# Berghojo/bmhrl

Measured on AMD Instinct MI355X. Metric: caption-train steps/sec, higher is better.
Workload: dtype bf16; 1 GPU; BMHRL warmstart step (BASELINE configs[1]): B=16/GPU Tv=256 Ta=800 L=30 V=10172 N=2 d_model=1024 H=4 dropout=0.1; global_batch=16, parallelism=dp1, launch=hip-graph

## Files before the change

### bmhrl_amd/_lib.py

```python
from __future__ import annotations

import ctypes as C
import os

_HERE = os.path.dirname(os.path.abspath(__file__))
LIB_PATH = os.environ.get("BMHRL_HIP_LIB") or os.path.join(_HERE, "csrc", "libbmhrl_hip.so")

i32, i64, u64, f32, f64 = C.c_int32, C.c_int64, C.c_uint64, C.c_float, C.c_double
ptr = C.c_void_p


class RnnLayer(C.Structure):
    _fields_ = [("w_ih", C.c_void_p), ("w_hh", C.c_void_p), ("b_ih", C.c_void_p), ("b_hh", C.c_void_p),
                ("in_seq", C.c_void_p), ("in_ld", C.c_int64), ("in_dim", C.c_int32), ("gates", C.c_int32),
                ("seq_out", C.c_void_p), ("h", C.c_void_p * 2), ("c", C.c_void_p * 2),
                ("arelu_alpha", C.c_void_p), ("arelu_beta", C.c_void_p), ("xproj", C.c_void_p)]


class FusionTailParams(C.Structure):
    _fields_ = [(n, C.c_void_p) for n in ("gamma_ca", "beta_ca", "gamma_cv", "beta_cv", "a_v",
                                          "dgamma_ca", "dbeta_ca", "dgamma_cv", "dbeta_cv", "da_v")]


class GemmDesc(C.Structure):
# ... 6 lines not shown
        ("epilogue", i32), ("alpha", f32), ("relu", i32), ("accumulate", i32), ("allow_split_k", i32),
        ("bias", ptr),
        ("residual", ptr), ("ldr", i64), ("r_sb1", i64), ("r_sb2", i64),
        ("mask", ptr), ("mask_sb1", i64), ("mask_sm", i64),
        ("rowvec", ptr), ("rowvec2", ptr), ("rv_sb1", i64), ("rv_sb2", i64),
        ("aux", ptr), ("ldaux", i64), ("aux_sb1", i64), ("aux_sb2", i64),
        ("dropout_p", f32), ("seed", u64), ("drop_sb1", i64), ("drop_sb2", i64), ("drop_sm", i64), ("seed_dev", ptr),
        ("colsum", ptr), ("colsum_sb2", i64), ("bias_sb2", i64), ("colsum_sb1", i64), ("bias_sb1", i64),
        ("split_ws", ptr), ("split_ws_elems", i64),
    ]


PROTOTYPES = {
    "bmhrl_gemm": [C.POINTER(GemmDesc), ptr],
    "bmhrl_gemm_group": [C.POINTER(GemmDesc), i32, ptr],
    "bmhrl_attention_fwd": [ptr, i64, ptr, i64, ptr, i64, ptr, i64, ptr, ptr, ptr, i64, i64, i32, i32, i32, i32, i32, f32,
                            f32, u64, ptr, ptr],
    "bmhrl_attention_shared128_fwd": [ptr, i64, ptr, i64, ptr, i64, ptr, ptr, ptr, i64, i32, i32, i32, i32, f32, ptr],
    "bmhrl_attention_fwd_f16": [ptr, i64, ptr, i64, ptr, i64, ptr, i64, ptr, ptr, ptr, i64, i64, i32, i32, i32, i32, i32, f32,
                                f32, u64, ptr, ptr],
    "bmhrl_attention_shared128_fwd_f16": [ptr, i64, ptr, i64, ptr, i64, ptr, ptr, ptr, i64, i32, i32, i32, i32, f32, ptr],
    "bmhrl_attention_shared128_bwd": [ptr, i64, ptr, i64, ptr, i64, ptr, ptr, ptr, ptr, i64, ptr, i64, ptr, i64, i32, ptr, i32, i32,
                                      i32, i32, f32, ptr],
    "bmhrl_small_attention_fwd": [ptr, i64, ptr, i64, ptr, i64, ptr, i64, ptr, i32, ptr, i64, i64, i32, i32, i32, i32, i32, f32, f32,
                                  u64, ptr, ptr],
    "bmhrl_small_attention_bwd": [ptr, i64, ptr, i32, ptr, i64, ptr, i64, ptr, i64, ptr, i64, ptr, i64, ptr, i64, ptr, ptr, ptr,
                                  ptr, i64, i64, i32, i32, i32, i32, i32, f32, ptr],
    "bmhrl_cast_memory": [ptr, ptr, ptr, i32, i32, i32, i32, ptr],
    "bmhrl_memory_attention": [i32, ptr, i64, ptr, i64, ptr, i64, i32, ptr, i64, i64, ptr, i64, ptr, i64, i32, i32, i32, i32, i32,
                               i32, f32, ptr],
    "bmhrl_softmax_rows": [ptr, i64, ptr, i64, i64, i32, i32, i64, ptr],
    "bmhrl_softmax_bwd_rows": [ptr, i64, ptr, i64, ptr, i64, i64, i32, f32, ptr, i64, i64, i32, i32, i32, i64, ptr],
    "bmhrl_attn_delta": [ptr, i64, ptr, i64, ptr, f32, i32, i32, i32, i32, ptr],
    "bmhrl_attention_bwd_scores256": [ptr, i64, ptr, i64, ptr, i64, ptr, i64, ptr, ptr, ptr, i64, ptr, ptr, i64, i32, i32, i32, i32,
                                      f32, ptr],
    "bmhrl_layernorm_fwd": [ptr, ptr, ptr, ptr, i64, ptr, ptr, ptr, i64, i32, ptr],
    "bmhrl_layernorm_bwd": [ptr, ptr, ptr, ptr, ptr, ptr, ptr, ptr, ptr, i64, i32, ptr],
    "bmhrl_layernorm_bwd_ws": [ptr, ptr, ptr, ptr, ptr, ptr, ptr, ptr, ptr, i64, i32, ptr, i64, ptr],
    "bmhrl_layernorm_fwd_groups": [ptr, ptr, ptr, ptr, i64, ptr, ptr, ptr, i64, i32, i32, ptr],
    "bmhrl_layernorm_bwd_groups": [ptr, ptr, ptr, ptr, ptr, ptr, ptr, ptr, ptr, i64, i32, i32, ptr],
    "bmhrl_add_posenc": [ptr, ptr, ptr, ptr, ptr, i64, i32, i32, i32, f32, u64, ptr, ptr],
    "bmhrl_embed_posenc": [ptr, ptr, f32, ptr, ptr, ptr, ptr, i32, i32, i32, f32, f32, u64, ptr, ptr],
    "bmhrl_embed_bwd": [ptr, ptr, f32, ptr, ptr, i32, i32, i32, f32, ptr],
    "bmhrl_cast_bf16": [ptr, i64, ptr, i64, i64, i32, f32, f32, u64, ptr, ptr],
    "bmhrl_cast_split3_bf16": [ptr, i64, ptr, i64, i64, i32, i64, i32, ptr, i64, i32, ptr],
    "bmhrl_cast_colsum_bf16": [ptr, i64, ptr, i64, i64, i32, f32, f32, u64, ptr, ptr, ptr],
# ... 149 lines not shown
```

### bmhrl_amd/csrc/attention128.hip

```cpp
#include "attention_bwd.h"

bool bmhrl_attn128_pair_ok(int B, int H, int Sq, int Sk);
int bmhrl_attn128_pair_fwd(const void* Qp, int64_t ldq, const void* X, int64_t ldx, void* ctx, int64_t ldo, float* row_max,
                           float* row_sum, const uint8_t* mask, int64_t mask_sb, int32_t B, int32_t H, int32_t Sq, int32_t Sk,
                           float scale, hipStream_t stream);

namespace {
int g_cfg128 = 0;
}

void bmhrl_attn128_set_cfg(int code) { g_cfg128 = code; }

int bmhrl_attn128_plan_fwd(int B, int H, int Sq, int Sk) {
  if (B <= 0 || H <= 0 || Sq <= 0 || Sk <= 0) return -22;
  const bool pair_served = bmhrl_attn128_pair_ok(B, H, Sq, Sk);
  const int code = g_cfg128 != 0 ? g_cfg128 : attn128_auto_code(B, H, Sq, Sk, pair_served);
  if (code == 14) return pair_served ? 14 : -22;
  if (code != 41 && code != 22 && code != 24) return -22;
  if (Sk > AttnCfg<128, 4, 1, 4, true>::MAX_SK || !attn_grid_ok(B, H, Sq, code / 10)) return -22;
  return code;
}
int bmhrl_attn128_plan_bwd(int B, int H, int Sq, int Sk) {
  if (B <= 0 || H <= 0 || Sq <= 0 || Sk <= 0 || Sk > AttnCfg<128, 4, 1, 4, true>::MAX_SK) return -22;
  const bool wide = attn128_bwd_wide(B, H, Sq);
  if (!attn_grid_ok(B, H, Sq, wide ? 4 : 2)) return -22;
  return wide ? 41 : 22;
}

extern "C" int bmhrl_attention_shared128_fwd(const void* Qp, int64_t ldq, const void* X, int64_t ldx, void* ctx, int64_t ldo,
                                             float* row_max, float* row_sum, const uint8_t* mask, int64_t mask_sb,
                                             int32_t B, int32_t H, int32_t Sq, int32_t Sk, float scale,
                                             bmhrl_stream_t stream) {
  return attention128_entry(Qp, ldq, X, ldx, ctx, ldo, row_max, row_sum, mask, mask_sb, B, H, Sq, Sk, scale, g_cfg128,
                            (hipStream_t)stream, bmhrl_attn128_pair_fwd, bmhrl_attn128_pair_ok);
}

extern "C" int64_t bmhrl_attention_shared128_bwd_workspace(int32_t B, int32_t H, int32_t Sk) {
  return (int64_t)B * H * Sk * 128;
}

extern "C" int bmhrl_attention_shared128_bwd(const void* Qp, int64_t ldq, const void* X, int64_t ldx, const void* dCx, int64_t lddo,
                                             const float* row_max, const float* row_sum, const float* delta,
                                             const uint8_t* mask, int64_t mask_sb, void* dQp, int64_t lddq, float* dX,
                                             int64_t lddx, int32_t accumulate_dx, float* workspace, int32_t B, int32_t H,
                                             int32_t Sq, int32_t Sk, float scale, bmhrl_stream_t stream) {
  constexpr int DK = 128;
  BMHRL_CHECK_ARG(Qp && X && dCx && row_max && row_sum && delta && dQp);
  BMHRL_CHECK_ARG(B > 0 && H > 0 && Sq > 0 && Sk > 0);
  BMHRL_CHECK_ARG(ldq % 8 == 0 && ldx % 8 == 0 && lddo % 8 == 0 && lddq % 8 == 0);
  BMHRL_CHECK_ARG(ldq >= (int64_t)H * DK && ldx >= DK && lddo >= (int64_t)H * DK && lddq >= (int64_t)H * DK);
  BMHRL_CHECK_ARG((((uintptr_t)Qp | (uintptr_t)X | (uintptr_t)dCx | (uintptr_t)dQp) & 15) == 0);
  BMHRL_CHECK_ARG((int64_t)Sk * ldx * 2 < (1ll << 31));
  BMHRL_CHECK_ARG(dX == nullptr || (workspace != nullptr && lddx >= DK && lddx % 4 == 0 && ((uintptr_t)dX & 15) == 0));
  AttnBwdArgs a;
  a.Q = (const bf16_t*)Qp; a.ldq = ldq; a.X = (const bf16_t*)X; a.ldx = ldx; a.dO = (const bf16_t*)dCx; a.lddo = lddo;
  a.dQ = (bf16_t*)dQp; a.lddq = lddq; a.dXp = workspace;
  a.row_max = row_max; a.row_sum = row_sum; a.delta = delta; a.mask = mask; a.mask_sb = mask_sb;
  a.B = B; a.H = H; a.Sq = Sq; a.Sk = Sk; a.scale = scale;
  hipStream_t s = (hipStream_t)stream;
  const bool wide = attn128_bwd_wide(B, H, Sq);
  const int qw = wide ? 4 : 2;
  if (Sk > AttnCfg<DK, 4, 1, 4, true>::MAX_SK) return -22;
  a.q_tiles = (Sq + 32 * qw - 1) / (32 * qw);
  BMHRL_CHECK_ARG((int64_t)B * H * a.q_tiles * H * a.q_tiles < (1ll << 32));
  a.per_b = H * a.q_tiles;
  a.map_mode = (B % 8 == 0) ? 0 : 2;
  a.magic_perb = div_magic((unsigned)a.per_b);
  a.magic_qt = div_magic((unsigned)a.q_tiles);
  a.magic_h = div_magic((unsigned)H);
  dim3 grid((unsigned)(B * H * a.q_tiles));
  if (wide) hipLaunchKernelGGL((attn_bwd_dq128_kernel<4, 1, 4>), grid, dim3(256), 0, s, a);
  else hipLaunchKernelGGL((attn_bwd_dq128_kernel<2, 2, 4>), grid, dim3(256), 0, s, a);
  if (dX != nullptr) {
    const int kblocks = (Sk + 32 * DX_WAVES - 1) / (32 * DX_WAVES);
    hipLaunchKernelGGL((attn_bwd_dx128_kernel<4>), dim3((unsigned)(B * H * kblocks)), dim3(64 * DX_WAVES), 0, s, a);
    const long total = (long)B * Sk * 32;
    hipLaunchKernelGGL(attn_bwd_dx_reduce_kernel, dim3((unsigned)((total + 255) / 256)), dim3(256), 0, s, (const float*)workspace, dX,
                       (long)lddx, B, H, Sk, accumulate_dx);
  }
  return hip_status(hipGetLastError());
}
```

### bmhrl_amd/csrc/attention_bwd.h

```cpp
#pragma once
#include "attention_fwd.h"

namespace {

template <int OFF>
__device__ __forceinline__ f32x4 asm_ldsf4(unsigned addr) {
  f32x4 r;
  asm volatile("ds_read_b128 %0, %1 offset:%2" : "=v"(r) : "v"(addr), "n"(OFF));
  return r;
}

struct AttnBwdArgs {
  const bf16_t* Q; long ldq;
  const bf16_t* X; long ldx;
  const bf16_t* dO; long lddo;
  bf16_t* dQ; long lddq;
  float* dXp;
  const float* row_max; const float* row_sum; const float* delta;
  const uint8_t* mask; long mask_sb;
  int B, H, Sq, Sk;
  float scale;
  int q_tiles, map_mode, per_b;
  unsigned magic_perb, magic_qt, magic_h;
};

template <int QW, int KW, int NS>
__global__ __launch_bounds__(64 * QW * KW, 2) void attn_bwd_dq128_kernel(const AttnBwdArgs p) {
  constexpr int DK = 128;
  using C = AttnCfg<DK, QW, KW, NS, true>;
  constexpr int NW = C::NW, NT = C::NT, BN = C::BN, VST = C::VST, ND = C::ND, NH = C::NH;
  static_assert(NS >= 3, "tile t+1 has landed at the end of iteration t while tile t+NS-1 is in flight");
  __shared__ __attribute__((aligned(16))) char smem_raw[C::LDS_BYTES];
  uint64_t* s_slow = reinterpret_cast<uint64_t*>(smem_raw + C::MAIN_BYTES);
  uint64_t* s_valid = s_slow + C::WORDS;
  bf16_t* smem = reinterpret_cast<bf16_t*>(smem_raw);
  const unsigned lds0 = (unsigned)(uintptr_t)(__attribute__((address_space(3))) char*)smem_raw;
  constexpr float LOG2E = 1.4426950408889634f;

  const int tid = threadIdx.x, lane = tid & 63;
  const int wave_s = __builtin_amdgcn_readfirstlane(tid >> 6);
  const int qi = wave_s / KW, ki = wave_s % KW;
  const int r32 = lane & 31, h = lane >> 5;
  const int g1 = (lane >> 4) & 1, q4 = (lane & 15) >> 2, p4 = lane & 3;
  int bh, qt;
  if (p.map_mode == 0) {
    const int xcd = blockIdx.x & 7, idx = blockIdx.x >> 3;
    const int q1 = fast_div(idx, p.per_b, p.magic_perb), rem = idx - q1 * p.per_b;
    const int hq = fast_div(rem, p.q_tiles, p.magic_qt);
    bh = (xcd + 8 * q1) * p.H + hq;
// ... 25 lines not shown
      static_for<0, GL>([&](auto i) {
        constexpr int I = decltype(i)::value;
        const int r = RPI * I + hi_;
        unsigned o = (unsigned)(r * (int)p.ldx * 2 + ((pch_ ^ swz(wrow + r)) << 4) - 1024 * (I & 3));
        asm volatile("" : "+v"(o));
        glds16<1024 * (I & 3)>(base + o, sdst + (I / 4) * 4 * RPI * DK);
      });
    } else {
      int hi_ = hi, pch_ = pch;
      asm volatile("" : "+v"(hi_), "+v"(pch_));
      static_for<0, GL>([&](auto i) {
        constexpr int I = decltype(i)::value;
        const int r = RPI * I + hi_;
        const int gr = min(k0 + wrow + r, p.Sk - 1);
        glds16<0>(Xgb + (unsigned)(gr * (int)p.ldx * 2 + ((pch_ ^ swz(wrow + r)) << 4)), sdst + RPI * I * DK);
      });
    }
  };
#pragma unroll
  for (int s = 0; s < NS - 1; ++s)
    if (s < nt_all) issue_x(s);

  bf16x8 qf[8], dof[8];
  {
    const long ro = ((long)b * p.Sq + (q_ok ? q_row : 0));
    const bf16_t* qp = p.Q + ro * p.ldq + hd * DK + 8 * h;
    const bf16_t* dp = p.dO + ro * p.lddo + hd * DK + 8 * h;
#pragma unroll
    for (int s = 0; s < 8; ++s) {
      qf[s] = q_ok ? *reinterpret_cast<const bf16x8*>(qp + 16 * s) : zero_bf16x8();
      dof[s] = q_ok ? *reinterpret_cast<const bf16x8*>(dp + 16 * s) : zero_bf16x8();
    }
  }
  float m2 = 0.f, invl_s = 0.f, dl_s = 0.f;
  if (q_ok) {
    const long si = ((long)b * p.H + hd) * p.Sq + q_row;
    m2 = p.row_max[si] * LOG2E;
    invl_s = p.scale / p.row_sum[si];
    dl_s = p.delta[si] * invl_s;
  }
  const int n_words = (nt_all * BN + 255) >> 8;
  for (int j = 0; j * NW < n_words; ++j) {
    const int i0 = 4 * (tid + NT * j);
    uint32_t v = 0x01010101u;
    if (mrow_b != nullptr && i0 < p.Sk) {
      if (mask_al4 && i0 + 4 <= p.Sk) {
        v = *reinterpret_cast<const uint32_t*>(mrow_b + i0);
      } else {
        v = 0;
#pragma unroll
        for (int e = 0; e < 4; ++e)
          if (i0 + e < p.Sk) v |= (uint32_t)mrow_b[i0 + e] << (8 * e);
      }
    }
    bool any_slow = false, any_valid = false;
#pragma unroll
    for (int e = 0; e < 4; ++e) {
      const bool keep = i0 + e < p.Sk && ((v >> (8 * e)) & 0xffu) != 0;
      any_slow |= !keep;
      any_valid |= keep;
    }
    const uint64_t bs = __ballot(any_slow), bv = __ballot(any_valid);
// ... 179 lines not shown
      const int srow = lane / CPRO, sch = lane % CPRO;
      const int q0 = qt * (32 * QW) + qi * 32;
      bf16x8 wout[NST];
#pragma unroll
      for (int i = 0; i < NST; ++i) wout[i] = *reinterpret_cast<const bf16x8*>(img + (RPS * i + srow) * ROWB + sch * 16);
      bf16_t* op = p.dQ + ((long)b * p.Sq + q0 + srow) * p.lddq + hd * DK + MY * 32 + sch * 8;
      const long ostep = (long)RPS * p.lddq;
#pragma unroll
      for (int i = 0; i < NST; ++i) {
        if (q0 + RPS * i + srow < p.Sq) *reinterpret_cast<bf16x8*>(op) = wout[i];
        op += ostep;
      }
    }
  });
}

constexpr int DX_WAVES = 4;
template <int NS>
struct DxCfg {
  static constexpr int TILE = 32 * 128 * 2;
  static constexpr int STAT = 3 * 64 * 4;
  static constexpr int STAGE = 2 * TILE + STAT;
  static constexpr int OUT = DX_WAVES * 32 * (512 + 16);
  static constexpr int LDS = cmax(NS * STAGE, OUT);
};

template <int NS>
__global__ __launch_bounds__(64 * DX_WAVES, 2) void attn_bwd_dx128_kernel(const AttnBwdArgs p) {
  constexpr int DK = 128;
  using C = DxCfg<NS>;
  __shared__ __attribute__((aligned(16))) char smem_raw[C::LDS];
  const unsigned lds0 = (unsigned)(uintptr_t)(__attribute__((address_space(3))) char*)smem_raw;
  constexpr float LOG2E = 1.4426950408889634f;
  const int tid = threadIdx.x, lane = tid & 63;
  const int wave_s = __builtin_amdgcn_readfirstlane(tid >> 6);
  const int r32 = lane & 31, h = lane >> 5;
  const int g1 = (lane >> 4) & 1, q4 = (lane & 15) >> 2, p4 = lane & 3;
  const int kblocks = (p.Sk + 32 * DX_WAVES - 1) / (32 * DX_WAVES);
  const int bh = blockIdx.x / kblocks, kb = blockIdx.x - bh * kblocks;
  const int b = bh / p.H, hd = bh - b * p.H;
  const int key = kb * (32 * DX_WAVES) + wave_s * 32 + r32;
  const bool key_in = key < p.Sk;
  const bool keep = key_in && (p.mask == nullptr || p.mask[(long)b * p.mask_sb + key] != 0);
  const int nqt = (p.Sq + 31) / 32;
  auto swz = [](int row) { return ((row & 3) << 2) | ((row >> 2) & 3); };

  const int hi = lane >> 4, pch = lane & 15;
// ... 9 lines not shown
      const int gr = min(q0 + r, p.Sq - 1);
      const int sc = (pch ^ swz(r)) << 4;
      __builtin_amdgcn_global_load_lds((const __attribute__((address_space(1))) void*)(Qgb + (long)gr * p.ldq * 2 + sc),
                                       (__attribute__((address_space(3))) void*)(st + (2 * wave_s + i) * 1024), 16, 0, 0);
      __builtin_amdgcn_global_load_lds((const __attribute__((address_space(1))) void*)(Dgb + (long)gr * p.lddo * 2 + sc),
                                       (__attribute__((address_space(3))) void*)(st + C::TILE + (2 * wave_s + i) * 1024), 16, 0, 0);
    }
    if (wave_s < 3) {
      const float* src = wave_s == 0 ? p.row_max : (wave_s == 1 ? p.row_sum : p.delta);
      const int gq = min(q0 + lane, p.Sq - 1);
      __builtin_amdgcn_global_load_lds((const __attribute__((address_space(1))) void*)(src + sbase + gq),
                                       (__attribute__((address_space(3))) void*)(st + 2 * C::TILE + wave_s * 256), 4, 0, 0);
    }
  };
  constexpr int PT = 5;
#pragma unroll
  for (int s = 0; s < NS - 1; ++s)
    if (s < nqt) issue(s);

  bf16x8 xf[8];
  {
    const bf16_t* xp = p.X + ((long)b * p.Sk + min(key, p.Sk - 1)) * p.ldx + 8 * h;
#pragma unroll
    for (int s = 0; s < 8; ++s) xf[s] = *reinterpret_cast<const bf16x8*>(xp + 16 * s);
  }
  f32x16 o[4];
#pragma unroll
  for (int d = 0; d < 4; ++d)
#pragma unroll
    for (int r = 0; r < 16; ++r) o[d][r] = 0.f;

  unsigned r_addr[8], t_addr[4][2];
#pragma unroll
  for (int st = 0; st < 8; ++st) r_addr[st] = lds0 + r32 * 256 + (((2 * st + h) ^ swz(r32)) << 4);
#pragma unroll
  for (int dd = 0; dd < 4; ++dd)
#pragma unroll
    for (int sec = 0; sec < 2; ++sec) {
      const int lc = 4 * dd + 2 * g1 + (p4 >> 1);
      const int pc = lc ^ ((q4 << 2) | ((h + 2 * sec) & 3));
      t_addr[dd][sec] = lds0 + (4 * h + q4) * 256 + (pc << 4) + ((p4 & 1) << 3);
    }
  const unsigned s_addr = lds0 + 2 * C::TILE + (4 * h) * 4;

  const float c_log2 = p.scale * LOG2E;
  const bool wave3 = wave_s == 3;
  asm volatile("s_waitcnt vmcnt(0)" ::: "memory");
  __builtin_amdgcn_s_barrier();
  asm volatile("" ::: "memory");
  for (int t = 0; t < nqt; ++t) {
    const bool more = t + NS - 1 < nqt;
    if (more) issue(t + NS - 1);
    const unsigned soff = (unsigned)(t % NS) * C::STAGE;
    bf16x8 af[8];
    f32x16 s_acc, dp_acc;
#pragma unroll
    for (int r = 0; r < 16; ++r) { s_acc[r] = 0.f; dp_acc[r] = 0.f; }
#pragma unroll
    for (int st = 0; st < 8; ++st) asm volatile("ds_read_b128 %0, %1 offset:0" : "=v"(af[st]) : "v"(r_addr[st] + soff));
    asm volatile("s_waitcnt lgkmcnt(0)" : "+v"(af[0]), "+v"(af[1]), "+v"(af[2]), "+v"(af[3]), "+v"(af[4]), "+v"(af[5]), "+v"(af[6]), "+v"(af[7]));
    BMHRL_SB();
    static_for<0, 8>([&](auto st_) { s_acc = __builtin_amdgcn_mfma_f32_32x32x16_bf16(af[decltype(st_)::value], xf[decltype(st_)::value], s_acc, 0, 0, 0); });
    BMHRL_SB();
#pragma unroll
    for (int st = 0; st < 8; ++st) asm volatile("ds_read_b128 %0, %1 offset:%2" : "=v"(af[st]) : "v"(r_addr[st] + soff), "n"(C::TILE));
    f32x4 smax[4], ssum[4], sdel[4];
    smax[0] = asm_ldsf4<0>(s_addr + soff);   smax[1] = asm_ldsf4<32>(s_addr + soff);
    smax[2] = asm_ldsf4<64>(s_addr + soff);  smax[3] = asm_ldsf4<96>(s_addr + soff);
    ssum[0] = asm_ldsf4<256>(s_addr + soff); ssum[1] = asm_ldsf4<288>(s_addr + soff);
    ssum[2] = asm_ldsf4<320>(s_addr + soff); ssum[3] = asm_ldsf4<352>(s_addr + soff);
    sdel[0] = asm_ldsf4<512>(s_addr + soff); sdel[1] = asm_ldsf4<544>(s_addr + soff);
    sdel[2] = asm_ldsf4<576>(s_addr + soff); sdel[3] = asm_ldsf4<608>(s_addr + soff);
    asm volatile("s_waitcnt lgkmcnt(12)" : "+v"(af[0]), "+v"(af[1]), "+v"(af[2]), "+v"(af[3]), "+v"(af[4]), "+v"(af[5]), "+v"(af[6]), "+v"(af[7]));
    BMHRL_SB();
    static_for<0, 8>([&](auto st_) { dp_acc = __builtin_amdgcn_mfma_f32_32x32x16_bf16(af[decltype(st_)::value], xf[decltype(st_)::value], dp_acc, 0, 0, 0); });
    asm volatile("s_waitcnt lgkmcnt(0)"
                 : "+v"(smax[0]), "+v"(smax[1]), "+v"(smax[2]), "+v"(smax[3]), "+v"(ssum[0]), "+v"(ssum[1]), "+v"(ssum[2]), "+v"(ssum[3]),
                   "+v"(sdel[0]), "+v"(sdel[1]), "+v"(sdel[2]), "+v"(sdel[3]));
    BMHRL_SB();
    bf16x8 tf[4][2];
    auto read_t = [&](const unsigned base) {
#pragma unroll
      for (int dd = 0; dd < 4; ++dd) {
        const unsigned a0 = t_addr[dd][0] + base, a1 = t_addr[dd][1] + base;
        tf[dd][0] = join8(asm_tr4<0>(a0), asm_tr4<8 * 256>(a1));
        tf[dd][1] = join8(asm_tr4<16 * 256>(a0), asm_tr4<24 * 256>(a1));
      }
    };
    read_t(soff + C::TILE);
    bf16x8 pb[2], dsb[2];
    const int q0 = t * 32 + 4 * h;
    const bool ragged = t * 32 + 32 > p.Sq;
#pragma unroll
    for (int g = 0; g < 4; ++g)
#pragma unroll
      for (int j = 0; j < 4; ++j) {
        const int r = 4 * g + j;
        const float rmax = smax[g][j];
        const float m2 = rmax * LOG2E;
        float invl = __builtin_amdgcn_rcpf(ssum[g][j]);
        if (ragged && q0 + 8 * g + j >= p.Sq) invl = 0.f;
        const float e = __builtin_amdgcn_exp2f(fmaf(s_acc[r], c_log2, -m2));
        const float pr = keep ? e * invl : (rmax == NEG_MASK ? invl : 0.f);
        const float dsv = keep ? pr * (dp_acc[r] - sdel[g][j]) * p.scale : 0.f;
        pb[r >> 3][r & 7] = (bf16_t)pr;
        dsb[r >> 3][r & 7] = (bf16_t)dsv;
      }
    asm volatile("s_waitcnt lgkmcnt(0)"
                 : "+v"(tf[0][0]), "+v"(tf[0][1]), "+v"(tf[1][0]), "+v"(tf[1][1]), "+v"(tf[2][0]), "+v"(tf[2][1]), "+v"(tf[3][0]), "+v"(tf[3][1]));
    BMHRL_SB();
    static_for<0, 8>([&](auto i_) {
      constexpr int I = decltype(i_)::value;
      o[I / 2] = __builtin_amdgcn_mfma_f32_32x32x16_bf16(tf[I / 2][I % 2], pb[I % 2], o[I / 2], 0, 0, 0);
    });
    BMHRL_SB();
    read_t(soff);
    asm volatile("s_waitcnt lgkmcnt(0)"
                 : "+v"(tf[0][0]), "+v"(tf[0][1]), "+v"(tf[1][0]), "+v"(tf[1][1]), "+v"(tf[2][0]), "+v"(tf[2][1]), "+v"(tf[3][0]), "+v"(tf[3][1]));
    BMHRL_SB();
    static_for<0, 8>([&](auto i_) {
      constexpr int I = decltype(i_)::value;
      o[I / 2] = __builtin_amdgcn_mfma_f32_32x32x16_bf16(tf[I / 2][I % 2], dsb[I % 2], o[I / 2], 0, 0, 0);
    });
    if (more && NS > 2) {
      if (wave3) asm volatile("s_waitcnt vmcnt(%0)" ::"n"((NS - 2) * (PT - 1)) : "memory");
      else asm volatile("s_waitcnt vmcnt(%0)" ::"n"((NS - 2) * PT) : "memory");
    } else {
      asm volatile("s_waitcnt vmcnt(0)" ::: "memory");
    }
    __builtin_amdgcn_s_barrier();
    asm volatile("" ::: "memory");
  }
  asm volatile("s_waitcnt vmcnt(0) lgkmcnt(0)" ::: "memory");
  __builtin_amdgcn_s_barrier();
  asm volatile("" ::: "memory");

  constexpr int ROWB = 512 + 16;
  char* img = smem_raw + wave_s * 32 * ROWB;
#pragma unroll
  for (int dd = 0; dd < 4; ++dd)
#pragma unroll
    for (int g = 0; g < 4; ++g) {
      f32x4 v;
#pragma unroll
      for (int j = 0; j < 4; ++j) v[j] = o[dd][4 * g + j];
      *reinterpret_cast<f32x4*>(img + r32 * ROWB + (dd * 32 + 8 * g + 4 * h) * 4) = v;
    }
  const int srow = lane >> 5, sch = lane & 31;
  const int k0 = kb * (32 * DX_WAVES) + wave_s * 32;
  float* outp = p.dXp + (((long)b * p.H + hd) * p.Sk + k0 + srow) * DK + sch * 4;
#pragma unroll
  for (int i = 0; i < 16; ++i) {
    const f32x4 v = *reinterpret_cast<const f32x4*>(img + (2 * i + srow) * ROWB + sch * 16);
    if (k0 + 2 * i + srow < p.Sk) *reinterpret_cast<f32x4*>(outp) = v;
// ... 21 lines not shown
```

### bmhrl_amd/functional.py

```python
from __future__ import annotations

import math
import itertools
import os
import weakref
from typing import Optional

import torch

from . import ops
from .ops import pad8

_BF16 = torch.bfloat16


class ShadowCache:

    def __init__(self):
        self.w = {}
        self.b = {}
        self.split = {}
        self.epoch = 0

    def invalidate(self):
# ... 744 lines not shown
        rows = B * L
        ldx, dmp, Skp = pad8(dq), pad8(dm), pad8(Sk)
        scale = 1.0 / math.sqrt(dk)
        need = ctx.needs_input_grad
        dy = dy.contiguous()
        w_q, w_k, w_v, w_o = SHADOWS.weight(wq), SHADOWS.weight(wk), SHADOWS.weight(wv), SHADOWS.weight(wo)
        zeros = torch.zeros if dmp != dm else torch.empty
        dyb, dbo = _cast_dy(dy, rows, dq, p_drop, s_res, need[11])
        dOb = torch.empty(rows, D, dtype=_BF16, device=dev)
        dbv = SCRATCH.f32(D, device=dev) if need[9] else None
        dwo, _ = _linear_bwd(dyb, ldx, rows, dq, Ob, D, D, w_o, need_dw=need[10], need_db=False, need_dx=True,
                             dx_bf16=dOb, lddxb=D, dx_drop=p_drop, dx_seed=s_attn, dx_colsum=dbv)
        dwv = None
        if need[8]:
            dwv = SCRATCH.f32(D, dm, device=dev, zero=not ops.gemm_overwrites(dk, dm, rows, H))
            ops.gemm(dOb, Cx, dk, dm, rows, lda=D, ldb=H * dmp, a_trans=True, b_trans=True, batch=(1, H), a_strides=(0, dk),
                     b_strides=(0, dmp), C_f32=dwv, ldc=dm, c_strides=(0, dk * dm), allow_split_k=True)
        dCx = zeros(rows, H * dmp, dtype=_BF16, device=dev)
        ops.gemm(dOb, w_v, rows, dm, dk, lda=D, ldb=w_v.shape[1], b_trans=True, batch=(1, H), a_strides=(0, dk),
                 b_strides=(0, dk * w_v.shape[1]), C_bf16=dCx, ldcb=H * dmp, cb_strides=(0, dmp))
        delta = None
        if flash:
            delta = torch.empty(B, H, L, device=dev)
            ops.attn_delta(dCx, H * dmp, Cx, H * dmp, delta, B, H, L, dmp)
        dQp = zeros(rows, H * dmp, dtype=_BF16, device=dev)
        dmem = None
        dxn = None
        if flash and FUSED_ATTN_BWD:
            if self_att:
                dxn = torch.empty(rows, dq, device=dev)
                target = dxn
            elif need[1]:
                dmem = torch.empty(B, Sk, dm, device=dev)
                target = dmem
            else:
                target = None
            ops.attention_shared128_bwd(Qp, memb, dCx, stats[0], stats[1], delta, m8, msb, dQp, target, False, B, H, L, Sk,
                                        scale, H * dmp, dmp, H * dmp, H * dmp, lddx=dm)
        else:
            dS = _padded_bf16(B * L * H, Sk, dev).view(B, L, H, Skp)
            pstr = (L * H * Skp, Skp)
            if flash:
                P = _padded_bf16(B * L * H, Sk, dev).view(B, L, H, Skp)
                ops.gemm(Qp, memb, L, Sk, dm, lda=H * dmp, ldb=dmp, batch=(B, H), a_strides=(L * H * dmp, dmp),
                         b_strides=(Sk * dmp, 0), C_bf16=P, ldcb=H * Skp, cb_strides=pstr, epilogue=ops.EPI_PROB, alpha=scale,
                         mask=m8, mask_sb1=msb, mask_sm=0, rowvec=stats[0], rowvec2=stats[1], rv_strides=(H * L, L))
                ops.gemm(dCx, memb, L, Sk, dm, lda=H * dmp, ldb=dmp, batch=(B, H), a_strides=(L * H * dmp, dmp),
                         b_strides=(Sk * dmp, 0), C_bf16=dS, ldcb=H * Skp, cb_strides=pstr, epilogue=ops.EPI_DSCORE, alpha=scale,
                         rowvec=delta, rv_strides=(H * L, L), aux=P, ldaux=H * Skp, aux_strides=pstr, mask=m8, mask_sb1=msb)
            else:
                P = stats[0]
                dP = torch.empty(B, L, H, Skp, device=dev)
                ops.gemm(dCx, memb, L, Sk, dm, lda=H * dmp, ldb=dmp, batch=(B, H), a_strides=(L * H * dmp, dmp),
                         b_strides=(Sk * dmp, 0), C_f32=dP, ldc=H * Skp, c_strides=pstr)
                ops.softmax_bwd_rows(P, Skp, dP, Skp, dS, Skp, B * L * H, Sk, scale, m8, msb, msq, H, L)
            def grad_mem(target, first_accumulates):
                ops.gemm(P, dCx, Sk, dm, L * H, lda=Skp, ldb=dmp, a_trans=True, b_trans=True, batch=(B, 1),
                         a_strides=(L * H * Skp, 0), b_strides=(L * H * dmp, 0), C_f32=target, ldc=dm, c_strides=(Sk * dm, 0),
                         accumulate=first_accumulates)
                ops.gemm(dS, Qp, Sk, dm, L * H, lda=Skp, ldb=dmp, a_trans=True, b_trans=True, batch=(B, 1),
                         a_strides=(L * H * Skp, 0), b_strides=(L * H * dmp, 0), C_f32=target, ldc=dm, c_strides=(Sk * dm, 0),
# ... 1246 lines not shown
```

### bmhrl_amd/ops.py

```python
from __future__ import annotations

import ctypes as C
import math
import os
from typing import Optional, Tuple

import numpy as np
import torch

from . import _lib

EPI_LINEAR, EPI_PROB, EPI_DSCORE, EPI_RELU_BWD = 0, 1, 2, 3


def pad8(n: int) -> int:
    return (n + 7) & ~7


def stream() -> int:
    return torch._C._cuda_getCurrentRawStream(torch.cuda.current_device())


_Tensor, _Parameter = torch.Tensor, torch.nn.Parameter
_TENSORS = frozenset((_Tensor, _Parameter))
# ... 187 lines not shown
def memory_attention(backward, X, x_off, ldx, mem, mem_t, ldt, PD, pd_row, pd_slot, Y, ldy, mask, mask_sb, n_mem, B2, H, L, Sk, dm,
                     scale):
    _launch("bmhrl_memory_attention", int(backward), _at(X, x_off), ldx, mem, Sk * dm, mem_t, dm * ldt, ldt, PD, pd_row, pd_slot,
            Y, ldy, mask, mask_sb, n_mem, B2, H, L, Sk, dm, scale)


def attention_shared128_fwd(Qp, X, ctx, row_max, row_sum, mask, mask_sb, B, H, Sq, Sk, scale, ldq, ldx, ldo):
    f16 = Qp.dtype == torch.float16
    if any((t.dtype == torch.float16) != f16 for t in (X, ctx)):
        raise RuntimeError("attention_shared128_fwd: Qp, X and ctx must share one 16-bit type")
    _launch("bmhrl_attention_shared128_fwd_f16" if f16 else "bmhrl_attention_shared128_fwd", Qp, ldq, X, ldx, ctx, ldo, row_max,
            row_sum, mask, mask_sb, B, H, Sq, Sk, scale)


def attention_shared128_bwd(Qp, X, dCx, row_max, row_sum, delta, mask, mask_sb, dQp, dX, accumulate_dx, B, H, Sq, Sk, scale,
                            ldq, ldx, lddo, lddq, lddx=128):
    ws = None
    if dX is not None:
        ws = torch.empty(int(_query("bmhrl_attention_shared128_bwd_workspace", B, H, Sk)), device=Qp.device)
    _launch("bmhrl_attention_shared128_bwd", Qp, ldq, X, ldx, dCx, lddo, row_max, row_sum, delta, mask, mask_sb, dQp, lddq, dX,
            lddx, int(bool(accumulate_dx)), ws, B, H, Sq, Sk, scale)


def softmax_bwd_rows(P, ldp, dP, lddp, dS, ldds, rows, cols, scale, mask=None, mask_sb=0, mask_sq=0, rows_per_query=1, queries=1,
                     rows_per_group=0, group_stride=0, p_off=0, ds_off=0):
    _launch("bmhrl_softmax_bwd_rows", _at(P, p_off), ldp, dP, lddp, _at(dS, ds_off), ldds, rows, cols, scale, mask, mask_sb,
            mask_sq, rows_per_query, queries, rows_per_group, group_stride)


def softmax_rows(S, lds, P, ldp, rows, cols, rows_per_group=0, group_stride=0, p_off=0):
    _launch("bmhrl_softmax_rows", S, lds, _at(P, p_off), ldp, rows, cols, rows_per_group, group_stride)


def attn_delta(dO, lddo, O, ldo, delta, B, H, Sq, dk, scale=1.0):
    _launch("bmhrl_attn_delta", dO, lddo, O, ldo, delta, scale, B, H, Sq, dk)


def attention_bwd_scores256_ok(Sq, Sk, dk, msq):
    return bool(_query("bmhrl_attention_bwd_scores256_ok", Sq, Sk, dk, msq))


def attention_bwd_scores256(Q, ldq, K, ldk, V, ldv, dO, lddo, row_max, row_sum, mask, msb, P, dS, ldp, B, H, Sq, Sk, scale,
                            q_off=0, k_off=0, v_off=0):
    _launch("bmhrl_attention_bwd_scores256", _at(Q, q_off), ldq, _at(K, k_off), ldk, _at(V, v_off), ldv, dO, lddo, row_max,
            row_sum, mask, msb, P, dS, ldp, B, H, Sq, Sk, scale)

# ... 964 lines not shown
```

### include/bmhrl_hip.h

```cpp
#ifndef BMHRL_HIP_H
#define BMHRL_HIP_H

#include <stdint.h>

#ifdef __cplusplus
extern "C" {
#endif

typedef void* bmhrl_stream_t;

enum {
  BMHRL_EPI_LINEAR = 0,
  BMHRL_EPI_PROB = 1,
  BMHRL_EPI_DSCORE = 2,
  BMHRL_EPI_RELU_BWD = 3
};

typedef struct bmhrl_gemm_desc {
  int32_t M, N, K;
  int32_t batch1, batch2;
  const void* A; int64_t lda, a_sb1, a_sb2; int32_t a_trans;
  const void* B; int64_t ldb, b_sb1, b_sb2; int32_t b_trans;
  float* C;  int64_t ldc, c_sb1, c_sb2;
  void* Cb;  int64_t ldcb, cb_sb1, cb_sb2;
// ... 27 lines not shown
                        void* O, int64_t ldo, float* row_max, float* row_sum, const uint8_t* mask, int64_t mask_sb,
                        int64_t mask_sq,
                        int32_t B, int32_t H, int32_t Sq, int32_t Sk, int32_t DK, float scale,
                        float dropout_p, uint64_t seed, const uint64_t* seed_dev, bmhrl_stream_t stream);

int bmhrl_attention_shared128_fwd(const void* Qp, int64_t ldq, const void* X, int64_t ldx, void* ctx, int64_t ldo,
                                  float* row_max, float* row_sum, const uint8_t* mask, int64_t mask_sb,
                                  int32_t B, int32_t H, int32_t Sq, int32_t Sk, float scale, bmhrl_stream_t stream);

int bmhrl_attention_fwd_f16(const void* Q, int64_t ldq, const void* K, int64_t ldk, const void* V, int64_t ldv,
                            void* O, int64_t ldo, float* row_max, float* row_sum, const uint8_t* mask, int64_t mask_sb,
                            int64_t mask_sq, int32_t B, int32_t H, int32_t Sq, int32_t Sk, int32_t DK, float scale,
                            float dropout_p, uint64_t seed, const uint64_t* seed_dev, bmhrl_stream_t stream);
int bmhrl_attention_shared128_fwd_f16(const void* Qp, int64_t ldq, const void* X, int64_t ldx, void* ctx, int64_t ldo,
                                      float* row_max, float* row_sum, const uint8_t* mask, int64_t mask_sb,
                                      int32_t B, int32_t H, int32_t Sq, int32_t Sk, float scale, bmhrl_stream_t stream);

int64_t bmhrl_attention_shared128_bwd_workspace(int32_t B, int32_t H, int32_t Sk);
int bmhrl_attention_shared128_bwd(const void* Qp, int64_t ldq, const void* X, int64_t ldx, const void* dCx, int64_t lddo,
                                  const float* row_max, const float* row_sum, const float* delta, const uint8_t* mask,
                                  int64_t mask_sb, void* dQp, int64_t lddq, float* dX, int64_t lddx, int32_t accumulate_dx,
                                  float* workspace, int32_t B, int32_t H, int32_t Sq, int32_t Sk, float scale,
                                  bmhrl_stream_t stream);

int bmhrl_attention_max_keys(void);

int bmhrl_attention_config(int32_t head_dim, int32_t code);

int bmhrl_attention_plan(int32_t kind, int32_t B, int32_t H, int32_t Sq, int32_t Sk, int64_t mask_sq);

int bmhrl_small_attention_ok(int32_t Sq, int32_t Sk, int32_t dk);
int bmhrl_small_attention_fwd(const void* Q, int64_t ldq, const void* K, int64_t ldk, const void* V, int64_t ldv, void* O,
                              int64_t ldo, void* P, int32_t ldp, const uint8_t* mask, int64_t mask_sb, int64_t mask_sq,
                              int32_t B, int32_t H, int32_t Sq, int32_t Sk, int32_t dk, float scale, float dropout_p,
                              uint64_t seed, const uint64_t* seed_dev, bmhrl_stream_t stream);
int bmhrl_small_attention_bwd(const void* dO, int64_t lddo, const void* P, int32_t ldp, const void* Q, int64_t ldq,
                              const void* K, int64_t ldk, const void* V, int64_t ldv, void* dQ, int64_t lddq, void* dK,
                              int64_t lddk, void* dV, int64_t lddv, float* dbq, float* dbk, float* dbv, const uint8_t* mask,
                              int64_t mask_sb, int64_t mask_sq, int32_t B, int32_t H, int32_t Sq, int32_t Sk, int32_t dk,
                              float scale, bmhrl_stream_t stream);

int bmhrl_memory_attention_ok(int32_t L, int32_t Sk, int32_t dm);
int bmhrl_cast_memory(const float* x, void* y, void* y_t, int32_t B, int32_t Sk, int32_t dm, int32_t ldt, bmhrl_stream_t stream);
int bmhrl_memory_attention(int32_t backward, const void* X, int64_t ldx, const void* mem, int64_t mem_sb, const void* mem_t,
                           int64_t mem_t_sb, int32_t ldt, void* PD, int64_t pd_row, int64_t pd_slot, void* Y, int64_t ldy,
                           const uint8_t* mask, int64_t mask_sb, int32_t n_mem, int32_t B2, int32_t H, int32_t L, int32_t Sk,
// ... 345 lines not shown
```

Before: 210.3 steps/s (one step = one B=16 batch on one GPU; whole-job aggregate over all GPUs).

## Fuse attention delta into the dQ backward kernel and simplify the dX softmax math

The shared-128 attention backward gains a context-aware variant. The dQ kernel computes the per-row delta (dO·O) itself and writes it out, so the separate attn_delta launch is skipped when FUSED_ATTN_BWD is set. The dX kernel now folds the per-row max, sum, mask and delta into combined constants staged in LDS, which removes per-element reciprocal and branch work. It also lets waves with no live keys only take part in the pipeline barriers. In exchange there are extra LDS space and writes per tile, and the new path depends on FUSED_ATTN_BWD being defined elsewhere.

```diff
diff --git a/bmhrl_amd/_lib.py b/bmhrl_amd/_lib.py
--- a/bmhrl_amd/_lib.py
+++ b/bmhrl_amd/_lib.py
@@ -52,6 +52,8 @@
     "bmhrl_attention_shared128_fwd_f16": [ptr, i64, ptr, i64, ptr, i64, ptr, ptr, ptr, i64, i32, i32, i32, i32, f32, ptr],
     "bmhrl_attention_shared128_bwd": [ptr, i64, ptr, i64, ptr, i64, ptr, ptr, ptr, ptr, i64, ptr, i64, ptr, i64, i32, ptr, i32, i32,
                                       i32, i32, f32, ptr],
+    "bmhrl_attention_shared128_bwd_ctx": [ptr, i64, ptr, i64, ptr, i64, ptr, i64, ptr, ptr, ptr, ptr, i64, ptr, i64, ptr, i64, i32,
+                                          ptr, i32, i32, i32, i32, f32, ptr],
     "bmhrl_small_attention_fwd": [ptr, i64, ptr, i64, ptr, i64, ptr, i64, ptr, i32, ptr, i64, i64, i32, i32, i32, i32, i32, f32, f32,
                                   u64, ptr, ptr],
     "bmhrl_small_attention_bwd": [ptr, i64, ptr, i32, ptr, i64, ptr, i64, ptr, i64, ptr, i64, ptr, i64, ptr, i64, ptr, ptr, ptr,
diff --git a/bmhrl_amd/csrc/attention128.hip b/bmhrl_amd/csrc/attention128.hip
--- a/bmhrl_amd/csrc/attention128.hip
+++ b/bmhrl_amd/csrc/attention128.hip
@@ -39,23 +39,26 @@
   return (int64_t)B * H * Sk * 128;
 }
 
-extern "C" int bmhrl_attention_shared128_bwd(const void* Qp, int64_t ldq, const void* X, int64_t ldx, const void* dCx, int64_t lddo,
-                                             const float* row_max, const float* row_sum, const float* delta,
-                                             const uint8_t* mask, int64_t mask_sb, void* dQp, int64_t lddq, float* dX,
-                                             int64_t lddx, int32_t accumulate_dx, float* workspace, int32_t B, int32_t H,
-                                             int32_t Sq, int32_t Sk, float scale, bmhrl_stream_t stream) {
+namespace {
+int attention128_bwd(const void* Qp, int64_t ldq, const void* X, int64_t ldx, const void* dCx, int64_t lddo, const void* Cx,
+                     int64_t ldcx, const float* row_max, const float* row_sum, float* delta, const uint8_t* mask,
+                     int64_t mask_sb, void* dQp, int64_t lddq, float* dX, int64_t lddx, int32_t accumulate_dx, float* workspace,
+                     int32_t B, int32_t H, int32_t Sq, int32_t Sk, float scale, bmhrl_stream_t stream) {
   constexpr int DK = 128;
+  const bool ctx = Cx != nullptr;
   BMHRL_CHECK_ARG(Qp && X && dCx && row_max && row_sum && delta && dQp);
   BMHRL_CHECK_ARG(B > 0 && H > 0 && Sq > 0 && Sk > 0);
   BMHRL_CHECK_ARG(ldq % 8 == 0 && ldx % 8 == 0 && lddo % 8 == 0 && lddq % 8 == 0);
   BMHRL_CHECK_ARG(ldq >= (int64_t)H * DK && ldx >= DK && lddo >= (int64_t)H * DK && lddq >= (int64_t)H * DK);
   BMHRL_CHECK_ARG((((uintptr_t)Qp | (uintptr_t)X | (uintptr_t)dCx | (uintptr_t)dQp) & 15) == 0);
+  BMHRL_CHECK_ARG(!ctx || (ldcx % 8 == 0 && ldcx >= (int64_t)H * DK && ((uintptr_t)Cx & 15) == 0));
   BMHRL_CHECK_ARG((int64_t)Sk * ldx * 2 < (1ll << 31));
   BMHRL_CHECK_ARG(dX == nullptr || (workspace != nullptr && lddx >= DK && lddx % 4 == 0 && ((uintptr_t)dX & 15) == 0));
   AttnBwdArgs a;
   a.Q = (const bf16_t*)Qp; a.ldq = ldq; a.X = (const bf16_t*)X; a.ldx = ldx; a.dO = (const bf16_t*)dCx; a.lddo = lddo;
   a.dQ = (bf16_t*)dQp; a.lddq = lddq; a.dXp = workspace;
   a.row_max = row_max; a.row_sum = row_sum; a.delta = delta; a.mask = mask; a.mask_sb = mask_sb;
+  a.Cx = (const bf16_t*)Cx; a.ldcx = ldcx; a.delta_out = delta;
   a.B = B; a.H = H; a.Sq = Sq; a.Sk = Sk; a.scale = scale;
   hipStream_t s = (hipStream_t)stream;
   const bool wide = attn128_bwd_wide(B, H, Sq);
@@ -69,8 +72,13 @@
   a.magic_qt = div_magic((unsigned)a.q_tiles);
   a.magic_h = div_magic((unsigned)H);
   dim3 grid((unsigned)(B * H * a.q_tiles));
-  if (wide) hipLaunchKernelGGL((attn_bwd_dq128_kernel<4, 1, 4>), grid, dim3(256), 0, s, a);
-  else hipLaunchKernelGGL((attn_bwd_dq128_kernel<2, 2, 4>), grid, dim3(256), 0, s, a);
+  if (wide) {
+    if (ctx) hipLaunchKernelGGL((attn_bwd_dq128_kernel<4, 1, 4, true>), grid, dim3(256), 0, s, a);
+    else hipLaunchKernelGGL((attn_bwd_dq128_kernel<4, 1, 4, false>), grid, dim3(256), 0, s, a);
+  } else {
+    if (ctx) hipLaunchKernelGGL((attn_bwd_dq128_kernel<2, 2, 4, true>), grid, dim3(256), 0, s, a);
+    else hipLaunchKernelGGL((attn_bwd_dq128_kernel<2, 2, 4, false>), grid, dim3(256), 0, s, a);
+  }
   if (dX != nullptr) {
     const int kblocks = (Sk + 32 * DX_WAVES - 1) / (32 * DX_WAVES);
     hipLaunchKernelGGL((attn_bwd_dx128_kernel<4>), dim3((unsigned)(B * H * kblocks)), dim3(64 * DX_WAVES), 0, s, a);
@@ -80,3 +88,24 @@
   }
   return hip_status(hipGetLastError());
 }
+}
+
+extern "C" int bmhrl_attention_shared128_bwd(const void* Qp, int64_t ldq, const void* X, int64_t ldx, const void* dCx, int64_t lddo,
+                                             const float* row_max, const float* row_sum, const float* delta,
+                                             const uint8_t* mask, int64_t mask_sb, void* dQp, int64_t lddq, float* dX,
+                                             int64_t lddx, int32_t accumulate_dx, float* workspace, int32_t B, int32_t H,
+                                             int32_t Sq, int32_t Sk, float scale, bmhrl_stream_t stream) {
+  return attention128_bwd(Qp, ldq, X, ldx, dCx, lddo, nullptr, 0, row_max, row_sum, const_cast<float*>(delta), mask, mask_sb, dQp,
+                          lddq, dX, lddx, accumulate_dx, workspace, B, H, Sq, Sk, scale, stream);
+}
+
+extern "C" int bmhrl_attention_shared128_bwd_ctx(const void* Qp, int64_t ldq, const void* X, int64_t ldx, const void* dCx,
+                                                 int64_t lddo, const void* Cx, int64_t ldcx, const float* row_max,
+                                                 const float* row_sum, float* delta, const uint8_t* mask, int64_t mask_sb,
+                                                 void* dQp, int64_t lddq, float* dX, int64_t lddx, int32_t accumulate_dx,
+                                                 float* workspace, int32_t B, int32_t H, int32_t Sq, int32_t Sk, float scale,
+                                                 bmhrl_stream_t stream) {
+  BMHRL_CHECK_ARG(Cx != nullptr);
+  return attention128_bwd(Qp, ldq, X, ldx, dCx, lddo, Cx, ldcx, row_max, row_sum, delta, mask, mask_sb, dQp, lddq, dX, lddx,
+                          accumulate_dx, workspace, B, H, Sq, Sk, scale, stream);
+}
diff --git a/bmhrl_amd/csrc/attention_bwd.h b/bmhrl_amd/csrc/attention_bwd.h
--- a/bmhrl_amd/csrc/attention_bwd.h
+++ b/bmhrl_amd/csrc/attention_bwd.h
@@ -17,6 +17,8 @@
   bf16_t* dQ; long lddq;
   float* dXp;
   const float* row_max; const float* row_sum; const float* delta;
+  const bf16_t* Cx; long ldcx;
+  float* delta_out;
   const uint8_t* mask; long mask_sb;
   int B, H, Sq, Sk;
   float scale;
@@ -24,7 +26,7 @@
   unsigned magic_perb, magic_qt, magic_h;
 };
 
-template <int QW, int KW, int NS>
+template <int QW, int KW, int NS, bool CTX>
 __global__ __launch_bounds__(64 * QW * KW, 2) void attn_bwd_dq128_kernel(const AttnBwdArgs p) {
   constexpr int DK = 128;
   using C = AttnCfg<DK, QW, KW, NS, true>;
@@ -96,6 +98,7 @@
     if (s < nt_all) issue_x(s);
 
   bf16x8 qf[8], dof[8];
+  float delta_row = 0.f;
   {
     const long ro = ((long)b * p.Sq + (q_ok ? q_row : 0));
     const bf16_t* qp = p.Q + ro * p.ldq + hd * DK + 8 * h;
@@ -104,6 +107,16 @@
     for (int s = 0; s < 8; ++s) {
       qf[s] = q_ok ? *reinterpret_cast<const bf16x8*>(qp + 16 * s) : zero_bf16x8();
       dof[s] = q_ok ? *reinterpret_cast<const bf16x8*>(dp + 16 * s) : zero_bf16x8();
+    }
+    if constexpr (CTX) {
+      const bf16_t* cp = p.Cx + ro * p.ldcx + hd * DK + 8 * h;
+#pragma unroll
+      for (int s = 0; s < 8; ++s) {
+        const bf16x8 cf = q_ok ? *reinterpret_cast<const bf16x8*>(cp + 16 * s) : zero_bf16x8();
+#pragma unroll
+        for (int j = 0; j < 8; ++j) delta_row = fmaf((float)dof[s][j], (float)cf[j], delta_row);
+      }
+      delta_row += __shfl_xor(delta_row, 32);
     }
   }
   float m2 = 0.f, invl_s = 0.f, dl_s = 0.f;
@@ -111,7 +124,12 @@
     const long si = ((long)b * p.H + hd) * p.Sq + q_row;
     m2 = p.row_max[si] * LOG2E;
     invl_s = p.scale / p.row_sum[si];
-    dl_s = p.delta[si] * invl_s;
+    if constexpr (CTX) {
+      if (h == 0 && ki == 0) p.delta_out[si] = delta_row;
+    } else {
+      delta_row = p.delta[si];
+    }
+    dl_s = delta_row * invl_s;
   }
   const int n_words = (nt_all * BN + 255) >> 8;
   for (int j = 0; j * NW < n_words; ++j) {
@@ -337,7 +355,9 @@
   static constexpr int STAT = 3 * 64 * 4;
   static constexpr int STAGE = 2 * TILE + STAT;
   static constexpr int OUT = DX_WAVES * 32 * (512 + 16);
-  static constexpr int LDS = cmax(NS * STAGE, OUT);
+  static constexpr int MAIN = cmax(NS * STAGE, OUT);
+  static constexpr int ROWC = 3 * 32 * 4;
+  static constexpr int LDS = MAIN + DX_WAVES * ROWC;
 };
 
 template <int NS>
@@ -393,7 +413,7 @@
   {
     const bf16_t* xp = p.X + ((long)b * p.Sk + min(key, p.Sk - 1)) * p.ldx + 8 * h;
 #pragma unroll
-    for (int s = 0; s < 8; ++s) xf[s] = *reinterpret_cast<const bf16x8*>(xp + 16 * s);
+    for (int s = 0; s < 8; ++s) xf[s] = keep ? *reinterpret_cast<const bf16x8*>(xp + 16 * s) : zero_bf16x8();
   }
   f32x16 o[4];
 #pragma unroll
@@ -412,13 +432,38 @@
       const int pc = lc ^ ((q4 << 2) | ((h + 2 * sec) & 3));
       t_addr[dd][sec] = lds0 + (4 * h + q4) * 256 + (pc << 4) + ((p4 & 1) << 3);
     }
-  const unsigned s_addr = lds0 + 2 * C::TILE + (4 * h) * 4;
+  const unsigned st_addr = lds0 + 2 * C::TILE + r32 * 4;
+  const unsigned w_addr = lds0 + C::MAIN + wave_s * C::ROWC + r32 * 4;
+  const unsigned n_addr = lds0 + C::MAIN + wave_s * C::ROWC + (4 * h) * 4, c_addr = n_addr + (keep ? 0 : 128);
+  constexpr float NO_WEIGHT = -1e30f;
+  const float key_scale = keep ? p.scale : 0.f;
 
   const float c_log2 = p.scale * LOG2E;
   const bool wave3 = wave_s == 3;
+  const bool wave_live = kb * (32 * DX_WAVES) + wave_s * 32 < p.Sk;
+  auto publish = [&](const bool more) {
+    if (more && NS > 2) {
+      if (wave3) asm volatile("s_waitcnt vmcnt(%0)" ::"n"((NS - 2) * (PT - 1)) : "memory");
+      else asm volatile("s_waitcnt vmcnt(%0)" ::"n"((NS - 2) * PT) : "memory");
+    } else {
+      asm volatile("s_waitcnt vmcnt(0)" ::: "memory");
+    }
+    __builtin_amdgcn_s_barrier();
+    asm volatile("" ::: "memory");
+  };
   asm volatile("s_waitcnt vmcnt(0)" ::: "memory");
   __builtin_amdgcn_s_barrier();
   asm volatile("" ::: "memory");
+  if (!wave_live) {
+    for (int t = 0; t < nqt; ++t) {
+      const bool more = t + NS - 1 < nqt;
+      if (more) issue(t + NS - 1);
+      publish(more);
+    }
+    asm volatile("s_waitcnt vmcnt(0) lgkmcnt(0)" ::: "memory");
+    __builtin_amdgcn_s_barrier();
+    return;
+  }
   for (int t = 0; t < nqt; ++t) {
     const bool more = t + NS - 1 < nqt;
     if (more) issue(t + NS - 1);
@@ -426,28 +471,40 @@
     bf16x8 af[8];
     f32x16 s_acc, dp_acc;
 #pragma unroll
-    for (int r = 0; r < 16; ++r) { s_acc[r] = 0.f; dp_acc[r] = 0.f; }
+    for (int r = 0; r < 16; ++r) s_acc[r] = 0.f;
+    float st_max, st_sum, st_del;
+    asm volatile("ds_read_b32 %0, %1 offset:0" : "=v"(st_max) : "v"(st_addr + soff));
+    asm volatile("ds_read_b32 %0, %1 offset:256" : "=v"(st_sum) : "v"(st_addr + soff));
+    asm volatile("ds_read_b32 %0, %1 offset:512" : "=v"(st_del) : "v"(st_addr + soff));
 #pragma unroll
     for (int st = 0; st < 8; ++st) asm volatile("ds_read_b128 %0, %1 offset:0" : "=v"(af[st]) : "v"(r_addr[st] + soff));
-    asm volatile("s_waitcnt lgkmcnt(0)" : "+v"(af[0]), "+v"(af[1]), "+v"(af[2]), "+v"(af[3]), "+v"(af[4]), "+v"(af[5]), "+v"(af[6]), "+v"(af[7]));
+    asm volatile("s_waitcnt lgkmcnt(0)"
+                 : "+v"(af[0]), "+v"(af[1]), "+v"(af[2]), "+v"(af[3]), "+v"(af[4]), "+v"(af[5]), "+v"(af[6]), "+v"(af[7]), "+v"(st_max),
+                   "+v"(st_sum), "+v"(st_del));
     BMHRL_SB();
     static_for<0, 8>([&](auto st_) { s_acc = __builtin_amdgcn_mfma_f32_32x32x16_bf16(af[decltype(st_)::value], xf[decltype(st_)::value], s_acc, 0, 0, 0); });
     BMHRL_SB();
+    {
+      const float lg = __builtin_amdgcn_logf(st_sum);
+      const bool past = t * 32 + r32 >= p.Sq;
+      const float ck = past ? NO_WEIGHT : -fmaf(st_max, LOG2E, lg);
+      const float cm = (past || st_max != NEG_MASK) ? NO_WEIGHT : -lg;
+      asm volatile("ds_write_b32 %0, %1 offset:0" ::"v"(w_addr), "v"(ck) : "memory");
+      asm volatile("ds_write_b32 %0, %1 offset:128" ::"v"(w_addr), "v"(cm) : "memory");
+      asm volatile("ds_write_b32 %0, %1 offset:256" ::"v"(w_addr), "v"(-st_del) : "memory");
+    }
 #pragma unroll
     for (int st = 0; st < 8; ++st) asm volatile("ds_read_b128 %0, %1 offset:%2" : "=v"(af[st]) : "v"(r_addr[st] + soff), "n"(C::TILE));
-    f32x4 smax[4], ssum[4], sdel[4];
-    smax[0] = asm_ldsf4<0>(s_addr + soff);   smax[1] = asm_ldsf4<32>(s_addr + soff);
-    smax[2] = asm_ldsf4<64>(s_addr + soff);  smax[3] = asm_ldsf4<96>(s_addr + soff);
-    ssum[0] = asm_ldsf4<256>(s_addr + soff); ssum[1] = asm_ldsf4<288>(s_addr + soff);
-    ssum[2] = asm_ldsf4<320>(s_addr + soff); ssum[3] = asm_ldsf4<352>(s_addr + soff);
-    sdel[0] = asm_ldsf4<512>(s_addr + soff); sdel[1] = asm_ldsf4<544>(s_addr + soff);
-    sdel[2] = asm_ldsf4<576>(s_addr + soff); sdel[3] = asm_ldsf4<608>(s_addr + soff);
-    asm volatile("s_waitcnt lgkmcnt(12)" : "+v"(af[0]), "+v"(af[1]), "+v"(af[2]), "+v"(af[3]), "+v"(af[4]), "+v"(af[5]), "+v"(af[6]), "+v"(af[7]));
+    f32x4 cr[4], nd[4];
+    cr[0] = asm_ldsf4<0>(c_addr);   cr[1] = asm_ldsf4<32>(c_addr);  cr[2] = asm_ldsf4<64>(c_addr);  cr[3] = asm_ldsf4<96>(c_addr);
+    nd[0] = asm_ldsf4<256>(n_addr); nd[1] = asm_ldsf4<288>(n_addr); nd[2] = asm_ldsf4<320>(n_addr); nd[3] = asm_ldsf4<352>(n_addr);
+    asm volatile("s_waitcnt lgkmcnt(0)"
+                 : "+v"(af[0]), "+v"(af[1]), "+v"(af[2]), "+v"(af[3]), "+v"(af[4]), "+v"(af[5]), "+v"(af[6]), "+v"(af[7]), "+v"(cr[0]),
+                   "+v"(cr[1]), "+v"(cr[2]), "+v"(cr[3]), "+v"(nd[0]), "+v"(nd[1]), "+v"(nd[2]), "+v"(nd[3]));
+#pragma unroll
+    for (int r = 0; r < 16; ++r) dp_acc[r] = nd[r >> 2][r & 3];
     BMHRL_SB();
     static_for<0, 8>([&](auto st_) { dp_acc = __builtin_amdgcn_mfma_f32_32x32x16_bf16(af[decltype(st_)::value], xf[decltype(st_)::value], dp_acc, 0, 0, 0); });
-    asm volatile("s_waitcnt lgkmcnt(0)"
-                 : "+v"(smax[0]), "+v"(smax[1]), "+v"(smax[2]), "+v"(smax[3]), "+v"(ssum[0]), "+v"(ssum[1]), "+v"(ssum[2]), "+v"(ssum[3]),
-                   "+v"(sdel[0]), "+v"(sdel[1]), "+v"(sdel[2]), "+v"(sdel[3]));
     BMHRL_SB();
     bf16x8 tf[4][2];
     auto read_t = [&](const unsigned base) {
@@ -460,22 +517,14 @@
     };
     read_t(soff + C::TILE);
     bf16x8 pb[2], dsb[2];
-    const int q0 = t * 32 + 4 * h;
-    const bool ragged = t * 32 + 32 > p.Sq;
 #pragma unroll
     for (int g = 0; g < 4; ++g)
 #pragma unroll
       for (int j = 0; j < 4; ++j) {
         const int r = 4 * g + j;
-        const float rmax = smax[g][j];
-        const float m2 = rmax * LOG2E;
-        float invl = __builtin_amdgcn_rcpf(ssum[g][j]);
-        if (ragged && q0 + 8 * g + j >= p.Sq) invl = 0.f;
-        const float e = __builtin_amdgcn_exp2f(fmaf(s_acc[r], c_log2, -m2));
-        const float pr = keep ? e * invl : (rmax == NEG_MASK ? invl : 0.f);
-        const float dsv = keep ? pr * (dp_acc[r] - sdel[g][j]) * p.scale : 0.f;
+        const float pr = __builtin_amdgcn_exp2f(fmaf(s_acc[r], c_log2, cr[g][j]));
         pb[r >> 3][r & 7] = (bf16_t)pr;
-        dsb[r >> 3][r & 7] = (bf16_t)dsv;
+        dsb[r >> 3][r & 7] = (bf16_t)(pr * dp_acc[r] * key_scale);
       }
     asm volatile("s_waitcnt lgkmcnt(0)"
                  : "+v"(tf[0][0]), "+v"(tf[0][1]), "+v"(tf[1][0]), "+v"(tf[1][1]), "+v"(tf[2][0]), "+v"(tf[2][1]), "+v"(tf[3][0]), "+v"(tf[3][1]));
@@ -493,14 +542,7 @@
       constexpr int I = decltype(i_)::value;
       o[I / 2] = __builtin_amdgcn_mfma_f32_32x32x16_bf16(tf[I / 2][I % 2], dsb[I % 2], o[I / 2], 0, 0, 0);
     });
-    if (more && NS > 2) {
-      if (wave3) asm volatile("s_waitcnt vmcnt(%0)" ::"n"((NS - 2) * (PT - 1)) : "memory");
-      else asm volatile("s_waitcnt vmcnt(%0)" ::"n"((NS - 2) * PT) : "memory");
-    } else {
-      asm volatile("s_waitcnt vmcnt(0)" ::: "memory");
-    }
-    __builtin_amdgcn_s_barrier();
-    asm volatile("" ::: "memory");
+    publish(more);
   }
   asm volatile("s_waitcnt vmcnt(0) lgkmcnt(0)" ::: "memory");
   __builtin_amdgcn_s_barrier();
diff --git a/bmhrl_amd/functional.py b/bmhrl_amd/functional.py
--- a/bmhrl_amd/functional.py
+++ b/bmhrl_amd/functional.py
@@ -790,7 +790,8 @@
         delta = None
         if flash:
             delta = torch.empty(B, H, L, device=dev)
-            ops.attn_delta(dCx, H * dmp, Cx, H * dmp, delta, B, H, L, dmp)
+            if not FUSED_ATTN_BWD:
+                ops.attn_delta(dCx, H * dmp, Cx, H * dmp, delta, B, H, L, dmp)
         dQp = zeros(rows, H * dmp, dtype=_BF16, device=dev)
         dmem = None
         dxn = None
@@ -803,8 +804,8 @@
                 target = dmem
             else:
                 target = None
-            ops.attention_shared128_bwd(Qp, memb, dCx, stats[0], stats[1], delta, m8, msb, dQp, target, False, B, H, L, Sk,
-                                        scale, H * dmp, dmp, H * dmp, H * dmp, lddx=dm)
+            ops.attention_shared128_bwd_ctx(Qp, memb, dCx, Cx, stats[0], stats[1], delta, m8, msb, dQp, target, False, B, H, L,
+                                            Sk, scale, H * dmp, dmp, H * dmp, H * dmp, H * dmp, lddx=dm)
         else:
             dS = _padded_bf16(B * L * H, Sk, dev).view(B, L, H, Skp)
             pstr = (L * H * Skp, Skp)
diff --git a/bmhrl_amd/ops.py b/bmhrl_amd/ops.py
--- a/bmhrl_amd/ops.py
+++ b/bmhrl_amd/ops.py
@@ -233,6 +233,15 @@
             lddx, int(bool(accumulate_dx)), ws, B, H, Sq, Sk, scale)
 
 
+def attention_shared128_bwd_ctx(Qp, X, dCx, Cx, row_max, row_sum, delta, mask, mask_sb, dQp, dX, accumulate_dx, B, H, Sq, Sk, scale,
+                                ldq, ldx, lddo, ldcx, lddq, lddx=128):
+    ws = None
+    if dX is not None:
+        ws = torch.empty(int(_query("bmhrl_attention_shared128_bwd_workspace", B, H, Sk)), device=Qp.device)
+    _launch("bmhrl_attention_shared128_bwd_ctx", Qp, ldq, X, ldx, dCx, lddo, Cx, ldcx, row_max, row_sum, delta, mask, mask_sb, dQp,
+            lddq, dX, lddx, int(bool(accumulate_dx)), ws, B, H, Sq, Sk, scale)
+
+
 def softmax_bwd_rows(P, ldp, dP, lddp, dS, ldds, rows, cols, scale, mask=None, mask_sb=0, mask_sq=0, rows_per_query=1, queries=1,
                      rows_per_group=0, group_stride=0, p_off=0, ds_off=0):
     _launch("bmhrl_softmax_bwd_rows", _at(P, p_off), ldp, dP, lddp, _at(dS, ds_off), ldds, rows, cols, scale, mask, mask_sb,
diff --git a/include/bmhrl_hip.h b/include/bmhrl_hip.h
--- a/include/bmhrl_hip.h
+++ b/include/bmhrl_hip.h
@@ -73,6 +73,11 @@
                                   int64_t mask_sb, void* dQp, int64_t lddq, float* dX, int64_t lddx, int32_t accumulate_dx,
                                   float* workspace, int32_t B, int32_t H, int32_t Sq, int32_t Sk, float scale,
                                   bmhrl_stream_t stream);
+int bmhrl_attention_shared128_bwd_ctx(const void* Qp, int64_t ldq, const void* X, int64_t ldx, const void* dCx, int64_t lddo,
+                                      const void* Cx, int64_t ldcx, const float* row_max, const float* row_sum, float* delta,
+                                      const uint8_t* mask, int64_t mask_sb, void* dQp, int64_t lddq, float* dX, int64_t lddx,
+                                      int32_t accumulate_dx, float* workspace, int32_t B, int32_t H, int32_t Sq, int32_t Sk,
+                                      float scale, bmhrl_stream_t stream);
 
 int bmhrl_attention_max_keys(void);
 
```

Result: no change. 211.7 steps/s (one step = one B=16 batch on one GPU; whole-job aggregate over all GPUs), median of 6 (+0.7%).
